# MarToonLi/StableDiffusionEO

Hardware: AMD Instinct MI355X
Metric: 512x512 canny2image images/sec (20 DDIM steps); ms per UNet step reported alongside (higher is better)
Workload: dtype f16; 1 GPU; SD1.5 + ControlNet-canny 512x512, batch=1 per GPU (CFG pair fused, N=2), 20 DDIM steps + VAE decode, fp16 storage / fp32 accumulate (BASELINE configs[1]); model_config=sd15, ddim_steps=20, parallelism=dp1 (image index -> rank, RCCL all_gather of final latents), weights=seeded synthetic (no checkpoint in the container)

## Files before the change

stablediffusioneo_amd/csrc/api_ops.hip:

```cpp
#include <stdarg.h>

#include "../../include/sdeo.h"
#include "sdeo_internal.h"
#include "kernels.h"

namespace sdeo {

static thread_local std::string g_last_error;

void set_error(const std::string& msg) { g_last_error = msg; }

int fail(const char* fmt, ...) {
  char buf[1024];
  va_list ap;
  va_start(ap, fmt);
  vsnprintf(buf, sizeof(buf), fmt, ap);
  va_end(ap);
  g_last_error = buf;
  return 1;
}

}

using namespace sdeo;
// ... 178 lines not shown
  (void)disarm_fp8();
  SDEO_CHECK(slots && groups > 0 && cout % groups == 0, "conv2d_gn: bad arguments");
  ConvGemm p;
  if (int rc = fill_conv(p, n, h, w, cin, cout, ksize, stride, upsample2x)) return rc;
  p.x = (const f16*)x; p.w = (const f16*)w_krsc; p.y = (f16*)y; p.bias = bias; p.res = (const f16*)res;
  p.bias2 = bias2; p.ld_bias2 = cout;
  const int cpg = cout / groups;
  *slots = conv_gemm_gn_slots(p, cpg);
  if (*slots <= 0) { *slots = 0; return 0; }
  const size_t need = (size_t)n * *slots * groups * 2, fold = *slots > 128 ? (size_t)n * groups * 2 : 0;
  SDEO_CHECK(partials && partial_floats >= need + fold, "conv2d_gn: partials buffer too small");
  p.gn_out = partials; p.gn_cpg = cpg; p.gn_slots = *slots; p.gn_groups = groups;
  if (int rc = conv_gemm(p, S(stream))) return rc;
  GnArgs g{(f16*)ynorm, (const f16*)y, gamma, beta, partials + need, cout, cout, n, p.Ho * p.Wo, cout, groups, eps, with_silu};
  g.ext_partials = partials; g.ext_nsc = *slots;
  return groupnorm_nhwc(g, S(stream));
}

static void fill_gemm(ConvGemm& p, int m, int n, int k) {
  p.B = m; p.Hi = p.Wi = p.Ho = p.Wo = 1; p.Cin = k; p.R = p.S = 1; p.stride = 1; p.pad = 0;
  p.M = m; p.N = n; p.K = k;
}

int sdeo_debug_gemm_plan(int m, int n, int k, int act, int fp8, int* key10, int* tile, int* splitk) {
  SDEO_CHECK(key10 && tile && splitk, "gemm_plan: null argument");
  ConvGemm p;
  fill_gemm(p, m, n, k);
  p.act = act;
  if (fp8) take_fp8(p, kQueryFp8);
  conv_gemm_query_plan(p, key10, tile, splitk);
// ... 280 lines not shown
```

stablediffusioneo_amd/csrc/kernels.h:

```cpp
#pragma once
#include <vector>

#include "common.h"

namespace sdeo {

struct ConvGemm {
  const f16* x = nullptr;
  const f16* w = nullptr;
  f16* y = nullptr;
  float* y32 = nullptr;
  const float* bias = nullptr;
  const float* bias2 = nullptr;
  const f16* res = nullptr;
  float* workspace = nullptr;
  size_t workspace_bytes = 0;
  int M = 0, N = 0, K = 0;
  int B = 1, Hi = 1, Wi = 1, Cin = 0;
  int Ho = 1, Wo = 1, R = 1, S = 1, stride = 1, pad = 0;
  int pad_after = -1;
  int ups = 0;
  int ldx = 0, ldw = 0, ldy = 0, ldres = 0, ld_bias2 = 0;
  int act = 0;
  int bias_per_row = 0;
// ... 55 lines not shown
int groupnorm_nhwc(f16* y, int ldy, const f16* x, int ldx, const float* gamma, const float* beta, int B, int HW, int C,
                   int groups, float eps, int with_silu, float* partials, hipStream_t stream);

struct GnArgs {
  f16* y; const f16* x; const float* gamma; const float* beta; float* partials;
  int ldy, ldx, B, HW, C, groups;
  float eps;
  int with_silu;
  const float* ext_partials = nullptr;
  int ext_nsc = 0;
};
bool groupnorm_is_single_launch(const GnArgs& a);
int gn_fused_threads(const GnArgs& a);
int groupnorm_nhwc(const GnArgs& a, hipStream_t stream);

int layernorm(f16* y, int ldy, const f16* x, int ldx, const float* gamma, const float* beta, int rows, int C, float eps,
              hipStream_t stream);

int attention(f16* o, int ldo, const f16* q, int ldq, const f16* k, int ldk, const f16* v, int ldv, int B, int H,
              int Tq, int Tk, int TkS, int TkSv, int d, float scale, hipStream_t stream, int causal = 0);
struct AttnArgs {
  f16* o; const f16* q; const f16* k; const f16* v;
  int ldo, ldq, ldk, ldv, B, H, Tq, Tk, TkS, TkSv, d;
  float scale;
  int causal;
  int qB = 0;
  int plan_B = 0;
};
int attention(const AttnArgs& a, hipStream_t stream);
const char* attention_kernel_name(int B, int H, int Tq, int Tk, int d, int causal);
// ... 74 lines not shown
```

stablediffusioneo_amd/csrc/net_build.hip:

```cpp
#include "net_handle.h"

namespace sdeo {

struct RowStats {
  float* p = nullptr;
  int ld = 0, strips = 0, c = 0;
};

struct ConvOpts {
  const float* bias2 = nullptr; int ld_bias2 = 0;
  const float* const* bias2_cur = nullptr; const int* ld_bias2_cur = nullptr; int bias2_off = 0;
  const T* res = nullptr;
  bool res_half = false;
  int act = 0;
  const float* scale_host = nullptr;
  const T* out = nullptr;
  int cout_store = -1;
  RowStats* stats = nullptr;
  const RowStats* ln = nullptr;
  const float* ln_s = nullptr;
  bool gn_next = false;
  const f16* w_ovr = nullptr; const float* b_ovr = nullptr;
  int pad_before = -1, pad_after = -1;
};

struct Builder {
  typedef ConvOpts CO;
  Engine* e;
  const Lane* lane;
  bool dry;
  bool share = false, half = false;
  Program* prog = nullptr;
  size_t max_splitk = 0, max_gn = 0;
  std::string err;

  T alloc(int n, int h, int w, int c) {
    T t;
    t.n = n; t.h = h; t.w = w; t.c = c; t.ld = c;
    t.off = lane->arena->alloc((size_t)n * h * w * c * 2);
    t.p = reinterpret_cast<f16*>(lane->base + t.off);
    return t;
  }
  T alloc2d(int rows, int c) { return alloc(1, 1, rows, c); }
  void release(T& t) { t.release(*lane->arena); }
  void advance(T& cur, T next) { release(cur); cur = next; }
  template <class F>
// ... 99 lines not shown
    T y = o.out ? o.out->view() : alloc(x.n, ho, wo, cs);
    const int n = half ? x.n / 2 : x.n;
    if (w && w->ipad != x.c && err.empty()) err = "conv " + name + ": input has " + std::to_string(x.c) + " channels, weight expects " + std::to_string(w->ipad);
    p.x = x.p; p.y = y.p;
    if (o.w_ovr) { p.w = o.w_ovr; p.bias = o.b_ovr; } else { p.w = wptr(name + ".weight"); p.bias = vptr(name + ".bias"); }
    p.bias2 = o.bias2; p.ld_bias2 = o.ld_bias2;
    if (o.res) { p.res = o.res->p; p.ldres = o.res->ld; }
    p.B = n; p.Hi = x.h; p.Wi = x.w; p.Cin = x.c; p.Ho = ho; p.Wo = wo; p.R = p.S = k; p.stride = stride; p.pad = pad; p.ups = ups;
    if (pad_after != pad) p.pad_after = pad_after;
    p.M = n * ho * wo; p.N = cs; p.K = k * k * x.c;
    if (half) p.plan_B = x.n;
    if (o.res_half) p.res_rows = p.M / 2;
    p.ldx = x.ld; p.ldw = p.K; p.ldy = y.ld; p.act = o.act;
    const bool want_gn = o.gn_next && !o.out && !o.scale_host && cs == y.c;
    if (want_gn) reserve_gn_partials(p, y);
    launch_conv(p, o.scale_host, o.stats, want_gn ? &y : nullptr, &o);
    return y;
  }

  T gemm(const T& x, const f16* w, int ldw, int n, const float* bias, const CO& o = CO(), float* out32 = nullptr, int ld32 = 0) {
    ConvGemm p;
    const int rows = half ? x.rows() / 2 : x.rows();
    T y;
    if (!out32) y = o.out ? o.out->view() : alloc(x.n, x.h, x.w, n);
    p.x = x.p; p.w = w; p.bias = bias;
    if (out32) { p.y32 = out32; p.ldy = ld32; } else { p.y = y.p; p.ldy = y.ld; }
    if (o.res) { p.res = o.res->p; p.ldres = o.res->ld; }
    p.B = rows; p.Cin = x.c; p.M = rows; p.N = n; p.K = x.c;
    p.ldx = x.ld; p.ldw = ldw; p.act = o.act;
    if (half) p.plan_B = x.rows();
    if (o.res_half) p.res_rows = rows / 2;
    set_ln(p, o);
// ... 21 lines not shown
    max_gn = std::max(max_gn, (size_t)B * gn_chunks(HW) * 32 * 2 * sizeof(float));
    const Lane* ws = lane;
    const f16* xp = x.p; f16* yp = y.p; const int ldx = x.ld, ldy = y.ld;
    GnArgs ga{yp, xp, g, b, nullptr, ldy, ldx, B, HW, C, 32, eps, silu_};
    const bool apply_only = x.gnp && !groupnorm_is_single_launch(ga);
    if (apply_only) {
      ga.ext_partials = x.gnp; ga.ext_nsc = x.gn_slots;
      max_gn = std::max(max_gn, (size_t)B * 32 * 2 * sizeof(float));
    }
    push([=](hipStream_t s) mutable { ga.partials = ws->gn_ws; return groupnorm_nhwc(ga, s); }, "groupnorm", 0,
         (apply_only ? 2.0 : 3.0) * 2.0 * B * HW * C, "C" + std::to_string(C) + " HW" + std::to_string(HW) + (apply_only ? " apply" : ""));
    return y;
  }

  T gn_conv(const T& x, const std::string& gn_name, float eps, int silu_, const std::string& conv_name, int cout, CO o) {
    T t = gn(x, gn_name, eps, silu_);
    T y = conv(t, conv_name, cout, 3, 1, 0, o);
    release(t);
    return y;
  }

  void attn(const T& o, const f16* q, int ldq, const f16* k, int ldk, const f16* v, int ldv, int B, int H, int Tq, int Tk, int TkS, int TkSv, int d,
            int qB = 0, const f16* k2 = nullptr, const f16* v2 = nullptr, int ldk2 = 0, int Tk2 = 0, int Tk2S = 0) {
    AttnArgs a{o.p, q, k, v, o.ld, ldq, ldk, ldv, B, H, Tq, Tk, TkS, TkSv, d, 1.0f / sqrtf((float)d), 0};
    a.qB = qB;
    if (half) { a.plan_B = B; a.B = B / 2; }
    B = a.B;
    const std::string tag = "Tq" + std::to_string(Tq) + " Tk" + std::to_string(Tk) + (k2 ? "+" + std::to_string(Tk2) : "") + " d" + std::to_string(d);
    if (k2) {
      if (!attention2_kernel_name(a.plan_B ? a.plan_B : a.B, H, Tq, Tk, Tk2, d) && err.empty()) err = std::string("image-prompt cross-attention: ") + sdeo_last_error();
      const Attn2Seg s2{k2, v2, ldk2, ldk2, Tk2, Tk2S, Tk2S, 0.f};
      const float* w = &e->ip_scale;
      push([=](hipStream_t s) { Attn2Seg x = s2; x.w = *w; return attention2(a, x, s); }, "attention",
           4.0 * B * H * (double)Tq * (Tk + Tk2) * d, 2.0 * B * H * d * (2.0 * Tq + 2.0 * (Tk + Tk2)), tag);
// ... 272 lines not shown
    if (i + 1 == e->hconvs.size()) o.out = &c.hint_feat[j];
    b.advance(x, b.conv(x, ns + hc.name, hc.cout, 3, hc.stride, 0, o));
  }
}

static T run_blocks(BuildCtx& c, const std::string& ns, const std::vector<Blk>& blocks, T x, bool release_in, int net, const T* final_out) {
  Builder& b = c.b;
  for (size_t i = 0; i < blocks.size(); ++i) {
    const Blk& blk = blocks[i];
    const T* out = (i + 1 == blocks.size()) ? final_out : nullptr;
    T y;
    switch (blk.kind) {
      case B_RES: y = build_res(b, ns, blk, x, net, out); break;
      case B_ATTN: y = build_attn(b, ns, blk, x, c.kv[net].at(ns + blk.name), net == 0 && b.e->ip_tokens ? &c.kv_ip.at(ns + blk.name) : nullptr, out); break;
      default: {
        Builder::CO o; o.out = out; o.gn_next = true;
        y = b.conv(x, ns + blk.name + conv_suffix(blk.kind), blk.cout, 3, blk.kind == B_DOWN ? 2 : 1, blk.kind == B_UP ? 1 : 0, o);
      }
    }
    if (release_in || i > 0) b.release(x);
    x = y;
  }
  return x;
}

struct Splice { size_t first = 0, last = 0; Program var; bool on = false; };
static T build_shared_prefix(BuildCtx& c, const std::string& ns, const std::vector<Blk>& blocks, const T& x, int net, Splice& sp) {
  Builder& b = c.b;
  Arena& arena = *b.lane->arena;
  const Arena before = arena;
  sp.first = b.prog->size();
// ... 24 lines not shown
  Builder& b = c.b; Engine* e = b.e;
  Splice sp;
  Program& p_cn = cn_prog(e, j, CP_CN);
  b.prog = &p_cn;
  const int net = 1 + j;
  const std::string ns = net_ns(net);
  auto zero_conv = [&](const T& x, const std::string& name, int cout, const T* out) {
    const size_t first = p_cn.size();
    Builder::CO zo; zo.out = out;
    b.conv(x, name, cout, 1, 1, 0, zo);
    for (size_t k = first; k < p_cn.size(); ++k) p_cn[k].zero_conv = true;
  };
  T hcur = e->x0;
  for (size_t i = 0; i < e->cplan.in.size(); ++i) {
    if (i == 0) {
      Builder::CO o; o.res = &c.hint_feat[j]; o.gn_next = true;
      hcur = b.conv(hcur, ns + e->cplan.in[0][0].name, e->cfg.model_channels, 3, 1, 0, o);
    } else if (i == 1) {
      hcur = build_shared_prefix(c, ns, e->cplan.in[i], hcur, net, sp);
    } else {
      hcur = run_blocks(c, ns, e->cplan.in[i], hcur, false, net, nullptr);
    }
    e->cn_h[j][i] = hcur;
    zero_conv(hcur, ns + "zero_convs." + std::to_string(i) + ".0", e->cplan.in_ch[i], &e->ctrl[i]);
  }
  T m = run_blocks(c, ns, e->cplan.mid, hcur, false, net, nullptr);
  e->cn_h[j][c.nctrl - 1] = m;
  zero_conv(m, ns + "middle_block_out.0", e->cplan.in_ch.back(), &e->ctrl[c.nctrl - 1]);
  splice(c, cn_prog(e, j, CP_CN_SH), p_cn, sp);
}

// ... 56 lines not shown
    }
    --ci;
    b.release(skip);
    const std::vector<Blk>& blocks = e->uplan.out[oi];
    if (oi + 1 < e->uplan.out.size()) {
      const T& nskip = hs.back();
      const int c_hn = blocks.back().cout;
      const int up = blocks.back().kind == B_UP ? 2 : 1;
      T ncat = b.alloc(cat.n, cat.h * up, cat.w * up, c_hn + nskip.c);
      const T nview = ncat.view(0, c_hn);
      run_blocks(c, ns, blocks, cat, true, 0, &nview);
      cat = ncat;
    } else {
      T y = run_blocks(c, ns, blocks, cat, true, 0, nullptr);
      Builder::CO oo; oo.cout_store = 4 * ((e->cfg.out_channels + 3) / 4);
      oo.out = &e->eps16;
      b.gn_conv(y, ns + "out.0", 1e-5f, 1, ns + "out.2", e->cfg.out_channels, oo);
      b.release(y);
    }
  }
}

static void build_unet_decoder_multi(BuildCtx& c, std::vector<T> hs, T cat0, T view0) {
  Builder& b = c.b; Engine* e = b.e;
  const std::string ns = NS_UNET;
  const size_t stages = e->uplan.out.size(), nh = hs.size();
  std::vector<T> cats{cat0};
  for (size_t oi = 0; oi + 1 < stages; ++oi) {
    const std::vector<Blk>& blocks = e->uplan.out[oi];
    const T& prev = cats.back();
    const int up = blocks.back().kind == B_UP ? 2 : 1;
// ... 21 lines not shown
  for (size_t oi = 0; oi < stages; ++oi, --ci) {
    const T& skip = hs[nh - 1 - oi];
    zero_conv(ci, "zero_convs." + std::to_string(ci) + ".0", cats[oi].view(cats[oi].c - skip.c, skip.c), skip);
  }
  if (!b.dry)
    for (int j = 0; j <= e->extra; ++j) b.prog->push_back(conv_gemm_multi_op(zc[j], kZeroConvTile, zs[j]));
  for (T& skip : hs) b.release(skip);
  for (size_t oi = 0; oi < stages; ++oi) {
    const std::vector<Blk>& blocks = e->uplan.out[oi];
    if (oi + 1 < stages) {
      const T nview = cats[oi + 1].view(0, blocks.back().cout);
      run_blocks(c, ns, blocks, cats[oi], true, 0, &nview);
    } else {
      T y = run_blocks(c, ns, blocks, cats[oi], true, 0, nullptr);
      Builder::CO oo; oo.cout_store = 4 * ((e->cfg.out_channels + 3) / 4);
      oo.out = &e->eps16;
      b.gn_conv(y, ns + "out.0", 1e-5f, 1, ns + "out.2", e->cfg.out_channels, oo);
      b.release(y);
    }
  }
}

static void build_unet(BuildCtx& c, bool with_ctrl) {
  Builder& b = c.b; Engine* e = b.e;
  b.prog = &e->prog[with_ctrl ? P_UNET_ENC : P_UNET_NOCTRL];
  const std::string ns = NS_UNET;
  std::vector<T> hs;
  T hcur = e->x0;
  Splice sp;
  for (size_t i = 0; i < e->uplan.in.size(); ++i) {
    hcur = (i == 1 && with_ctrl) ? build_shared_prefix(c, ns, e->uplan.in[i], hcur, 0, sp) : run_blocks(c, ns, e->uplan.in[i], hcur, false, 0, nullptr);
// ... 89 lines not shown
  b.advance(hcur, b.gn_conv(hcur, d + ".norm_out", 1e-6f, 1, d + ".conv_out", 2 * zc, oo));
  b.advance(hcur, b.conv(hcur, std::string(NS_VAE) + "quant_conv", 2 * zc, 1, 1, 0, oo));
  float* zp = e->enc_z; float* mp = e->enc_moments; const float* np_ = e->enc_noise; const int* with_noise = &e->enc_with_noise;
  const f16* qp = hcur.p; const int ld = hcur.ld, HW = h * w; const float sf = cfg.vae_scale_factor;
  b.push([=](hipStream_t s) { return vae_posterior(zp, mp, qp, ld, *with_noise ? np_ : nullptr, zc, HW, sf, s); }, "vae_posterior", 0,
         (2.0 * 2 * zc + 4.0 * 4 * zc) * HW);
  b.release(hcur);
}

}

int sdeo::build_all(Engine* e, bool dry, size_t* max_splitk, size_t* max_gn, size_t peaks[L_COUNT]) {
  Arena arenas[L_COUNT];
  for (int i = 0; i < L_COUNT; ++i) e->lanes[i].arena = &arenas[i];
  BuildCtx c{Builder{e, &e->lanes[L_MAIN], dry}, e->N, e->lh, e->lw, round8(e->cfg.context_len), (int)e->cplan.in.size() + 1};
  build_persistent(c);
  build_latent_io(c);
  build_time_embeds(c);
  for (int net = 0; net < 2 + e->extra; ++net) build_context(c, net);
  if (e->ip_tokens) build_context_ip(c);
  for (int j = 0; j <= e->extra; ++j) build_hint(c, j);
  c.b.on_lane(&e->lanes[L_SIDE], [&] { for (int j = 0; j <= e->extra; ++j) build_controlnet(c, j); });
  build_control_io(c);
  for (int variant = 0; variant < 2; ++variant) build_unet(c, variant == 0);
  build_vae_decoder(c);
  if (e->vae_encoder) build_vae_encoder(c);
  for (int i = 0; i < L_COUNT; ++i) {
    e->lanes[i].arena = nullptr;
    peaks[i] = align_up(arenas[i].peak, 256);
  }
// ... 5 lines not shown
```

stablediffusioneo_amd/csrc/norm.hip:

```cpp
#include <stdlib.h>

#include "kernels.h"

namespace sdeo {

struct GnOne {
  f16* y; const f16* x; const float* gamma; const float* beta; float* partials; int ldy, ldx;
};
struct GnPair { GnOne k[1]; };

int gn_chunks(int HW) { const int c = cdiv(HW, 8); return c > 128 ? 128 : (c < 1 ? 1 : c); }

static int gn_vec_per_block(int C, int groups) {
  const int nvec = C / 8, cpg = C / groups;
  for (int parts = 1; parts <= nvec; ++parts) {
    if (nvec % parts) continue;
    const int nvb = nvec / parts;
    if (nvb > 256) continue;
    if ((nvb * 8) % cpg) continue;
    return nvb;
  }
  return 0;
}

// ... 426 lines not shown
  if (chunks > 2048) chunks = 2048;
  const int ppc = cdiv(HW, chunks);
  dim3 grid(chunks, parts, B * count);
  int sc = cdiv(HW, 8 * P);
  { const int mxs = gn_chunks(HW) < 128 ? gn_chunks(HW) : 128; sc = sc < 1 ? 1 : (sc > mxs ? mxs : sc); }
  const int sppc = cdiv(HW, sc);
  dim3 sgrid(sc, parts, B * count);
  hipLaunchKernelGGL(gn_stats_kernel, sgrid, dim3(256), 0, stream, gp, B, HW, C, cpg, nvb, sc, groups, sppc);
  hipLaunchKernelGGL(gn_apply_kernel, grid, dim3(256), 0, stream, gp, B, HW, C, cpg, nvb, chunks, groups, eps, with_silu, ppc, sc);
  SDEO_HIP(hipGetLastError());
  return 0;
}

static GnOne gn_one(const GnArgs& a) { return GnOne{a.y, a.x, a.gamma, a.beta, a.partials, a.ldy, a.ldx}; }

int groupnorm_nhwc(const GnArgs& a, hipStream_t stream) {
  if (int rc = gn_check(a)) return rc;
  GnPair gp{};
  gp.k[0] = gn_one(a);
  return gn_dispatch(a, gp, 1, stream);
}

int groupnorm_nhwc(f16* y, int ldy, const f16* x, int ldx, const float* gamma, const float* beta, int B, int HW, int C,
                   int groups, float eps, int with_silu, float* partials, hipStream_t stream) {
  return groupnorm_nhwc(GnArgs{y, x, gamma, beta, partials, ldy, ldx, B, HW, C, groups, eps, with_silu}, stream);
}

template <int VPL>
__global__ __launch_bounds__(256) void layernorm_kernel(f16* __restrict__ y, int ldy, const f16* __restrict__ x, int ldx,
                                                        const float* __restrict__ gamma, const float* __restrict__ beta,
// ... 100 lines not shown
```

stablediffusioneo_amd/csrc/sdeo_internal.h:

```cpp
#ifndef SDEO_INTERNAL_H
#define SDEO_INTERNAL_H

#include <stdint.h>

#ifdef __cplusplus
extern "C" {
#endif

void sdeo_debug_force_gemm_plan(int tile, int splitk);
void sdeo_debug_force_gemm_order(int order);
const char* sdeo_debug_conv2d_kernel_name(int n, int h, int w, int cin, int cout, int ksize, int stride, int upsample2x);
const char* sdeo_debug_attention_kernel_name(int B, int H, int Tq, int Tk, int d, int causal);
const char* sdeo_debug_attention2_kernel_name(int B, int H, int Tq, int Tk, int Tk2, int d);
int sdeo_debug_attention2_check(void* o, int ldo, const void* q, int ldq, const void* k, int ldk, const void* v, int ldv, int tk, int tk_stride,
                                int v_batch_stride, const void* k2, int ldk2, const void* v2, int ldv2, int tk2, int tk2_stride,
                                int v2_batch_stride, float weight2, int b, int heads, int tq, int d, float scale);
int sdeo_debug_conv2d_plan(int n, int h, int w, int cin, int cout, int ksize, int stride, int upsample2x, int act, int fp8, int* key10,
                           int* tile, int* splitk);
int sdeo_debug_gemm_plan(int m, int n, int k, int act, int fp8, int* key10, int* tile, int* splitk);
int sdeo_debug_gemm_multi_f16(int count, const int* tile, const int* splitk, const int* m, const int* n, const int* k, void* const* y,
                              const int* ldy, const void* const* x, const int* ldx, const void* const* w, const int* ldw,
                              const void* const* bias, const void* const* res, const int* ldres, const float* scale, void* stream);
void sdeo_debug_last_gemm_plan(int* tile, int* splitk);
int sdeo_debug_last_gemm_epilogue(void);
// ... 17 lines not shown
int sdeo_debug_compose_proj(void* w_out, float* b_out, const void* wp, const float* bp, const void* w2, const float* b2, int c, int k2,
                            void* stream);
int sdeo_debug_gemm_stats_f16(void* y, int ldy, const void* x, int ldx, const void* w, int ldw, const float* bias, const void* res,
                              int ldres, int m, int n, int k, float* stats, int stats_ld, int* strips_out, void* stream);
int sdeo_debug_gemm_ln_f16(void* y, int ldy, const void* x, int ldx, const void* w_folded, int ldw, const float* ln_s,
                           const float* bias_folded, const float* stats, int stats_ld, int strips, int ln_c, int m, int n, int k, int act, float eps, void* workspace, size_t workspace_bytes, void* stream);
int sdeo_debug_row_stats_f16(float* stats, int stats_ld, const void* x, int ldx, int rows, int c, void* stream);
int sdeo_debug_conv2d_gn_f16(void* ynorm, void* y, const void* x, const void* w_krsc, const float* bias, const void* res, int n, int h,
                             int w, int cin, int cout, int ksize, int stride, int upsample2x, const float* gamma, const float* beta,
                             int groups, float eps, int with_silu, float* partials, size_t partial_floats, int* slots, void* stream);
int sdeo_debug_conv2d_gn_b2_f16(void* ynorm, void* y, const void* x, const void* w_krsc, const float* bias, const float* bias2, const void* res,
                                int n, int h, int w, int cin, int cout, int ksize, int stride, int upsample2x, const float* gamma,
                                const float* beta, int groups, float eps, int with_silu, float* partials, size_t partial_floats, int* slots,
                                void* stream);

int sdeo_debug_gemm_res_rows_f16(void* y, int ldy, const void* x, int ldx, const void* w, int ldw, const float* bias, const void* res,
                                 int ldres, int res_rows, int m, int n, int k, float* stats, int stats_ld, int* strips_out, void* workspace,
                                 size_t workspace_bytes, void* stream);
int sdeo_debug_conv2d_ex_f16(void* y, const void* x, const void* w_krsc, const float* bias, const void* res, int res_rows, int n, int h,
                             int w, int cin, int cout, int ksize, float* stats, int stats_ld, int* strips_out, const float* ln_stats,
                             const float* ln_s, int ln_ld, int ln_strips, void* workspace, size_t workspace_bytes, void* stream);
int sdeo_debug_attention_qb_f16(void* o, int ldo, const void* q, int ldq, const void* k, int ldk, const void* v, int ldv, int b,
                                int q_batches, int heads, int tq, int tk, int tk_stride, int v_batch_stride, int d, float scale, void* stream);
int sdeo_debug_attention2_qb_f16(void* o, int ldo, const void* q, int ldq, const void* k, int ldk, const void* v, int ldv, int tk,
                                 int tk_stride, int v_batch_stride, const void* k2, int ldk2, const void* v2, int ldv2, int tk2,
                                 int tk2_stride, int v2_batch_stride, float weight2, int b, int q_batches, int heads, int tq, int d,
                                 float scale, void* stream);

int sdeo_debug_quantize_mx(void* q_out, void* scales_out, const void* x, int rows, int cols, void* stream);
int sdeo_debug_gemm_mx_f16(void* y, int ldy, const void* xq, const void* xs, const void* wq, const void* ws, const float* bias, const void* res,
// ... 17 lines not shown
```

stablediffusioneo_amd/ops.py:

```python
from __future__ import annotations

import ctypes as C

import torch

from . import _lib
from ._lib import check, cur_stream, ptr


def _need_cuda(*ts):
    for t in ts:
        if t is not None and not t.is_cuda:
            raise _lib.SdeoError("HIP ops need device tensors (no CPU fallback)")


def _ws(nbytes, device):
    return torch.empty(max(int(nbytes), 16), dtype=torch.uint8, device=device)


def _nhwc_ld(t, what):
    n, h, w, _ = t.shape
    ld = t.stride(2)
    assert t.dtype == torch.float16 and t.stride(3) == 1 and (h == 1 or t.stride(1) == w * ld) and (n == 1 or t.stride(0) == h * w * ld), \
        f"groupnorm: {what} must be fp16 NHWC with unit channel stride and densely stacked pixels (shape {tuple(t.shape)}, strides {t.stride()})"
# ... 132 lines not shown
    hv, wv = (2 * h, 2 * w) if upsample2x else (h, w)
    pad = k // 2
    ho = (hv + 2 * pad - k) // stride + 1
    wo = (wv + 2 * pad - k) // stride + 1
    y = torch.empty((n, ho, wo, cout), dtype=torch.float16, device=x.device)
    yn = torch.empty_like(y)
    pf = n * (ho * wo) * groups * 2 // 16 + n * groups * 2 + 1024
    part = torch.empty(pf, dtype=torch.float32, device=x.device)
    slots = C.c_int(0)
    check(lib.sdeo_debug_conv2d_gn_f16(ptr(yn), ptr(y), ptr(x), ptr(w_krsc), ptr(bias), ptr(res), n, h, w, cin, cout, k, stride,
                                       int(upsample2x), ptr(gamma), ptr(beta), groups, eps, int(swish), ptr(part), pf, C.byref(slots),
                                       cur_stream()), "conv2d_gn")
    if slots.value == 0:
        return None
    return y, yn, slots.value


def gemm(x, w, bias=None, res=None, act=0, scale=1.0, out_f32=False, bias_per_row=False, w8=None, out=None):
    lib = _lib.load()
    _need_cuda(x, w)
    m, k = x.shape
    n, k2 = w.shape
    assert k == k2 and x.stride(1) == 1 and w.stride(1) == 1
    y = _out(out, (m, n), torch.float32 if out_f32 else torch.float16, x.device)
    nb = lib.sdeo_gemm_workspace_bytes(m, n, k)
    ws = _ws(nb if w8 is None else max(nb, 64 << 20), x.device)
    _arm_fp8(lib, w8)
    check(lib.sdeo_gemm_f16(ptr(y), n, ptr(x), x.stride(0), ptr(w), w.stride(0), ptr(bias), ptr(res),
                            res.stride(0) if res is not None else 0, m, n, k, act, scale, int(out_f32), int(bias_per_row), ptr(ws),
                            ws.numel(), cur_stream()), "gemm")
# ... 386 lines not shown
```

Baseline: 8.757 images/s.

## Add thin-channel conv kernels for UNet conv_in and fused GN-SiLU conv_out

Adds two specialised 3x3 conv kernels for the degenerate channel counts at the UNet and ControlNet edges. The first handles 4-to-8 stored input channels with the filter held in LDS and fdot2 accumulation, replacing the implicit-GEMM path. The second fuses GroupNorm finalisation, SiLU, and a 3x3 conv producing 4 output channels over a halo tile, with a cross-channel LDS reduction. Both are enabled by default through SDEO_THIN_CONVS. The goal is to avoid poorly utilised GEMM tiles and the separate normalised-tensor round trip, at the cost of new code paths and a large LDS footprint.

```diff
diff --git a/stablediffusioneo_amd/csrc/api_ops.hip b/stablediffusioneo_amd/csrc/api_ops.hip
--- a/stablediffusioneo_amd/csrc/api_ops.hip
+++ b/stablediffusioneo_amd/csrc/api_ops.hip
@@ -216,6 +216,31 @@
   if (int rc = conv_gemm(p, S(stream))) return rc;
   GnArgs g{(f16*)ynorm, (const f16*)y, gamma, beta, partials + need, cout, cout, n, p.Ho * p.Wo, cout, groups, eps, with_silu};
   g.ext_partials = partials; g.ext_nsc = *slots;
+  return groupnorm_nhwc(g, S(stream));
+}
+
+int sdeo_debug_conv3x3_cin4_f16(void* y, const void* x, const void* w_krsc, const float* bias, const void* res, int n_run, int h, int w, int cin,
+                                int cout, void* stream) {
+  const ThinConvIn a{(f16*)y, (const f16*)x, (const f16*)w_krsc, bias, (const f16*)res, cout, 8, 72, cout, n_run, h, w, cin, 8, cout};
+  return conv3x3_cin4(a, S(stream));
+}
+
+int sdeo_debug_gn_silu_conv3x3_cout4_f16(void* y, const void* x, const void* w_krsc, const float* bias, const float* gamma, const float* beta,
+                                         const float* partials, int slots, int n, int h, int w, int c, int cout, int groups, float eps,
+                                         int with_silu, void* workspace, void* stream) {
+  ThinConvOut a{(f16*)y, (const f16*)x, (const f16*)w_krsc, bias, gamma, beta, nullptr, 4, c, 9 * c, n, h, w, c, cout, groups, 0, eps, with_silu};
+  const char* why = gn_silu_conv3x3_cout4_refusal(a);
+  SDEO_CHECK(!why, "gn_silu_conv3x3_cout4: %s", why);
+  GnArgs g{nullptr, (const f16*)x, gamma, beta, (float*)workspace, c, c, n, h * w, c, groups, eps, with_silu};
+  if (partials) { g.ext_partials = partials; g.ext_nsc = slots; }
+  if (int rc = groupnorm_partials(g, &a.partials, &a.nsc, S(stream))) return rc;
+  return gn_silu_conv3x3_cout4(a, S(stream));
+}
+
+int sdeo_debug_groupnorm_from_partials_f16(void* y, const void* x, const float* gamma, const float* beta, const float* partials, int slots, int n,
+                                           int hw, int c, int groups, float eps, int with_silu, void* workspace, void* stream) {
+  GnArgs g{(f16*)y, (const f16*)x, gamma, beta, (float*)workspace, c, c, n, hw, c, groups, eps, with_silu};
+  g.ext_partials = partials; g.ext_nsc = slots;
   return groupnorm_nhwc(g, S(stream));
 }
 
diff --git a/stablediffusioneo_amd/csrc/conv_thin.hip b/stablediffusioneo_amd/csrc/conv_thin.hip
--- /dev/null
+++ b/stablediffusioneo_amd/csrc/conv_thin.hip
@@ -0,0 +1,341 @@
+#include "kernels.h"
+
+namespace sdeo {
+
+typedef _Float16 h2_t __attribute__((ext_vector_type(2)));
+typedef unsigned u32x4 __attribute__((ext_vector_type(4)));
+
+__device__ __forceinline__ float dot2(unsigned a, unsigned b, float c) {
+  return __builtin_amdgcn_fdot2(__builtin_bit_cast(h2_t, a), __builtin_bit_cast(h2_t, b), c, false);
+}
+
+template <int NP>
+struct PixVec { typedef unsigned type __attribute__((ext_vector_type(NP))); };
+
+template <int NP>
+__global__ __launch_bounds__(256) void conv3x3_cin4_kernel(const ThinConvIn a) {
+  kernarg_warm<sizeof(ThinConvIn)>();
+  typedef typename PixVec<NP>::type pix_t;
+  extern __shared__ __attribute__((aligned(16))) char thin_smem[];
+  pix_t* wl = reinterpret_cast<pix_t*>(thin_smem);
+  pix_t* tile = wl + a.Cout * 9;
+  const f16* __restrict__ x = a.x;
+  const f16* __restrict__ wgt = a.w;
+  const f16* __restrict__ res = a.res;
+  f16* __restrict__ y = a.y;
+  const int W = a.W, HW = a.H * a.W, L = a.L, ldx = a.ldx, ldy = a.ldy, ldres = a.ldres, ldw = a.ldw, cs = a.cin_store;
+  const int tid = threadIdx.x;
+  const int nvb = a.Cout >> 3, P = 256 / nvb;
+  const int cv = tid % nvb, prow = tid / nvb;
+  const bool active = prow < P;
+  const int b = blockIdx.y, p0 = blockIdx.x * L;
+  const int n = min(L, HW - p0);
+  const size_t img = (size_t)b * HW;
+
+#pragma unroll 4
+  for (int g = tid; g < a.Cout * 9; g += 256) {
+    const int row = g / 9, t = g - row * 9;
+    const u32x4 v = *reinterpret_cast<const u32x4*>(wgt + (size_t)row * ldw + t * cs);
+    pix_t o;
+#pragma unroll
+    for (int q = 0; q < NP; ++q) o[q] = v[q];
+    wl[((row & 7) * 9 + t) * nvb + (row >> 3)] = o;
+  }
+  const int nt = n + 2 * W + 2;
+  for (int i = tid; i < nt; i += 256) {
+    const int gp = p0 - W - 1 + i;
+    pix_t v = {};
+    if (gp >= 0 && gp < HW) v = *reinterpret_cast<const pix_t*>(x + (img + gp) * ldx);
+    tile[i] = v;
+  }
+  f32x4 bs[2] = {};
+  f16x8 rv[8];
+  if (active) {
+    if (a.bias) {
+      bs[0] = *reinterpret_cast<const f32x4*>(a.bias + cv * 8);
+      bs[1] = *reinterpret_cast<const f32x4*>(a.bias + cv * 8 + 4);
+    }
+    if (res) {
+#pragma unroll
+      for (int it = 0; it < 8; ++it) {
+        const int p = prow + it * P;
+        if (p < n) rv[it] = *reinterpret_cast<const f16x8*>(res + (img + p0 + p) * ldres + cv * 8);
+      }
+    }
+  }
+  __syncthreads();
+  if (!active) return;
+  pix_t w[8][9];
+#pragma unroll
+  for (int j = 0; j < 8; ++j)
+#pragma unroll
+    for (int t = 0; t < 9; ++t) w[j][t] = wl[(j * 9 + t) * nvb + cv];
+#pragma unroll
+  for (int it = 0; it < 8; ++it) {
+    const int p = prow + it * P;
+    if (p < n) {
+      const int xx = (p0 + p) % W;
+      float acc[8];
+#pragma unroll
+      for (int j = 0; j < 8; ++j) acc[j] = 0.f;
+#pragma unroll
+      for (int dy = 0; dy < 3; ++dy)
+#pragma unroll
+        for (int dx = 0; dx < 3; ++dx) {
+          pix_t v = tile[p + dy * W + dx];
+          if ((unsigned)(xx + dx - 1) >= (unsigned)W) v = pix_t{};
+#pragma unroll
+          for (int j = 0; j < 8; ++j)
+#pragma unroll
+            for (int q = 0; q < NP; ++q) acc[j] = dot2(v[q], w[j][dy * 3 + dx][q], acc[j]);
+        }
+      f16x8 o;
+#pragma unroll
+      for (int j = 0; j < 8; ++j) {
+        float f = acc[j] + bs[j >> 2][j & 3];
+        if (res) f += (float)rv[it][j];
+        o[j] = (f16)f;
+      }
+      *reinterpret_cast<f16x8*>(y + (img + p0 + p) * ldy + cv * 8) = o;
+    }
+  }
+}
+
+static int thin_conv_in_strip(const ThinConvIn& a) {
+  const int P = 256 / (a.Cout / 8), HW = a.H * a.W;
+  int L = cdiv(a.B * HW, 256);
+  L = L < P ? P : L;
+  L = L > 8 * P ? 8 * P : L;
+  L = L > 1024 ? 1024 : L;
+  return L > HW ? HW : L;
+}
+
+const char* conv3x3_cin4_refusal(const ThinConvIn& a) {
+  if (!a.y || !a.x || !a.w) return "null operand";
+  if (a.B < 1 || a.H < 1 || a.W < 1 || a.W > 1024) return "image size";
+  if (a.cin < 1 || a.cin > 8 || a.cin_store != 8 || a.ldw < 9 * a.cin_store) return "more than 8 stored input channels";
+  if (a.Cout < 8 || a.Cout % 8 || a.Cout > 384) return "output channels are no multiple of 8 (or above 384: the filter stays in LDS)";
+  if (a.ldx % 8 || a.ldy % 8 || a.ldw % 8 || (a.res && a.ldres % 8)) return "row strides are no multiples of 8";
+  if ((reinterpret_cast<uintptr_t>(a.x) | reinterpret_cast<uintptr_t>(a.y) | reinterpret_cast<uintptr_t>(a.w) | reinterpret_cast<uintptr_t>(a.res)) & 15)
+    return "operands are not 16-byte aligned";
+  if (a.bias && (reinterpret_cast<uintptr_t>(a.bias) & 15)) return "bias is not 16-byte aligned";
+  return nullptr;
+}
+
+int conv3x3_cin4(const ThinConvIn& a0, hipStream_t stream) {
+  const char* why = conv3x3_cin4_refusal(a0);
+  SDEO_CHECK(!why, "conv3x3_cin4: %s", why);
+  ThinConvIn a = a0;
+  a.L = thin_conv_in_strip(a);
+  const int HW = a.H * a.W, np = a.cin <= 4 ? 2 : 4;
+  const dim3 grid(cdiv(HW, a.L), a.B);
+  const size_t smem = (size_t)(a.Cout * 9 + a.L + 2 * a.W + 2) * np * 4;
+  SDEO_CHECK(smem <= 64 * 1024, "conv3x3_cin4: Cout=%d W=%d need %zu bytes of LDS", a.Cout, a.W, smem);
+  if (np == 2) hipLaunchKernelGGL(conv3x3_cin4_kernel<2>, grid, dim3(256), smem, stream, a);
+  else hipLaunchKernelGGL(conv3x3_cin4_kernel<4>, grid, dim3(256), smem, stream, a);
+  SDEO_HIP(hipGetLastError());
+  return 0;
+}
+
+static const int kThinPrefetch = 10;
+
+__global__ __launch_bounds__(256) void gn_silu_conv3x3_cout4_kernel(const ThinConvOut a) {
+  kernarg_warm<sizeof(ThinConvOut)>();
+  extern __shared__ __attribute__((aligned(16))) char thin_smem[];
+  const f16* __restrict__ x = a.x;
+  const f16* __restrict__ wgt = a.w;
+  const float* __restrict__ gamma = a.gamma;
+  const float* __restrict__ beta = a.beta;
+  const float* __restrict__ partials = a.partials;
+  f16* __restrict__ y = a.y;
+  const int H = a.H, W = a.W, C = a.C, ldx = a.ldx, ldw = a.ldw, TW = a.TW, TH = a.TH, groups = a.groups, nsc = a.nsc;
+  const int tid = threadIdx.x;
+  const int nvb = C >> 3, P = 256 / nvb;
+  const int cv = tid % nvb, prow = tid / nvb;
+  const bool active = prow < P;
+  const int b = blockIdx.y;
+  const int tx0 = (blockIdx.x % a.tiles_x) * TW, ty0 = (blockIdx.x / a.tiles_x) * TH;
+  const int HWD = TW + 2, HP = (TH + 2) * HWD, TP = TW * TH;
+  const int cpg = C / groups;
+  const int nab = C > 256 ? C : 256;
+  f16* halo = reinterpret_cast<f16*>(thin_smem);
+  f32x4* red = reinterpret_cast<f32x4*>(thin_smem + (size_t)HP * C * 2);
+  float* s_a = reinterpret_cast<float*>(red + (size_t)nvb * (TP + 1));
+  float* s_b = s_a + nab;
+  float* s_mean = s_b + nab;
+  float* s_rstd = s_mean + 64;
+  const f16* xb = x + (size_t)b * H * W * ldx + cv * 8;
+
+  f16x8 xv[kThinPrefetch];
+#pragma unroll
+  for (int u = 0; u < kThinPrefetch; ++u) {
+    const int hp = prow + u * P;
+    const int gy = ty0 + hp / HWD - 1, gx = tx0 + hp % HWD - 1;
+    xv[u] = f16x8{};
+    if (active && hp < HP && (unsigned)gy < (unsigned)H && (unsigned)gx < (unsigned)W)
+      xv[u] = *reinterpret_cast<const f16x8*>(xb + ((size_t)gy * W + gx) * ldx);
+  }
+  u32x4 w[4][9];
+#pragma unroll
+  for (int co = 0; co < 4; ++co)
+#pragma unroll
+    for (int t = 0; t < 9; ++t) {
+      w[co][t] = u32x4{};
+      if (active && co < a.cout) w[co][t] = *reinterpret_cast<const u32x4*>(wgt + (size_t)co * ldw + t * C + cv * 8);
+    }
+  float gpre[8], bpre[8];
+#pragma unroll
+  for (int k = 0; k < 8; ++k) {
+    const int c = tid + k * 256;
+    if (c < C) { gpre[k] = gamma[c]; bpre[k] = beta[c]; }
+  }
+  {
+    const int tpg = 256 / groups;
+    const int gl = tid / tpg, l = tid - gl * tpg;
+    float ts = 0.f, tq = 0.f;
+    if (gl < groups) {
+      const float2* src = reinterpret_cast<const float2*>(partials) + ((size_t)b * nsc * groups + gl);
+      for (int c0 = l; c0 < nsc; c0 += 8 * tpg) {
+        float2 v[8];
+#pragma unroll
+        for (int u = 0; u < 8; ++u) {
+          const int c = c0 + u * tpg;
+          v[u] = c < nsc ? src[(size_t)c * groups] : make_float2(0.f, 0.f);
+        }
+#pragma unroll
+        for (int u = 0; u < 8; ++u) { ts += v[u].x; tq += v[u].y; }
+      }
+    }
+    s_a[tid] = ts;
+    s_b[tid] = tq;
+  }
+  __syncthreads();
+  if (tid < groups) {
+    const int tpg = 256 / groups;
+    float ts = 0.f, tq = 0.f;
+    for (int l = 0; l < tpg; ++l) { ts += s_a[tid * tpg + l]; tq += s_b[tid * tpg + l]; }
+    const float inv = 1.0f / ((float)cpg * (float)(H * W));
+    const float mean = ts * inv;
+    float var = tq * inv - mean * mean;
+    var = var < 0.f ? 0.f : var;
+    s_mean[tid] = mean;
+    s_rstd[tid] = rsqrtf(var + a.eps);
+  }
+  __syncthreads();
+#pragma unroll
+  for (int k = 0; k < 8; ++k) {
+    const int c = tid + k * 256;
+    if (c < C) {
+      const int g = c / cpg;
+      const float sc = s_rstd[g] * gpre[k];
+      s_a[c] = sc;
+      s_b[c] = bpre[k] - s_mean[g] * sc;
+    }
+  }
+  __syncthreads();
+  if (active) {
+    float sa[8], sb[8];
+#pragma unroll
+    for (int j = 0; j < 8; ++j) { sa[j] = s_a[cv * 8 + j]; sb[j] = s_b[cv * 8 + j]; }
+    auto norm = [&](const f16x8& v, bool inside) {
+      f16x8 o;
+#pragma unroll
+      for (int j = 0; j < 8; ++j) {
+        float f = (float)v[j] * sa[j] + sb[j];
+        if (a.with_silu) f = silu_f(f);
+        o[j] = inside ? (f16)f : (f16)0.f;
+      }
+      return o;
+    };
+#pragma unroll
+    for (int u = 0; u < kThinPrefetch; ++u) {
+      const int hp = prow + u * P;
+      if (hp < HP) {
+        const int gy = ty0 + hp / HWD - 1, gx = tx0 + hp % HWD - 1;
+        *reinterpret_cast<f16x8*>(halo + (size_t)hp * C + cv * 8) = norm(xv[u], (unsigned)gy < (unsigned)H && (unsigned)gx < (unsigned)W);
+      }
+    }
+    for (int hp = prow + kThinPrefetch * P; hp < HP; hp += P) {
+      const int gy = ty0 + hp / HWD - 1, gx = tx0 + hp % HWD - 1;
+      const bool inside = (unsigned)gy < (unsigned)H && (unsigned)gx < (unsigned)W;
+      f16x8 v = {};
+      if (inside) v = *reinterpret_cast<const f16x8*>(xb + ((size_t)gy * W + gx) * ldx);
+      *reinterpret_cast<f16x8*>(halo + (size_t)hp * C + cv * 8) = norm(v, inside);
+    }
+  }
+  __syncthreads();
+  if (active) {
+    for (int p = prow; p < TP; p += P) {
+      const int py = p / TW, px = p - py * TW;
+      if (ty0 + py >= H || tx0 + px >= W) continue;
+      float acc[4] = {0.f, 0.f, 0.f, 0.f};
+#pragma unroll
+      for (int dy = 0; dy < 3; ++dy)
+#pragma unroll
+        for (int dx = 0; dx < 3; ++dx) {
+          const u32x4 v = *reinterpret_cast<const u32x4*>(halo + (size_t)((py + dy) * HWD + px + dx) * C + cv * 8);
+#pragma unroll
+          for (int co = 0; co < 4; ++co)
+#pragma unroll
+            for (int q = 0; q < 4; ++q) acc[co] = dot2(v[q], w[co][dy * 3 + dx][q], acc[co]);
+        }
+      red[(size_t)cv * (TP + 1) + p] = f32x4{acc[0], acc[1], acc[2], acc[3]};
+    }
+  }
+  __syncthreads();
+  if (tid < TP) {
+    const int py = tid / TW, px = tid - py * TW;
+    const int gy = ty0 + py, gx = tx0 + px;
+    if (gy < H && gx < W) {
+      f32x4 s = {0.f, 0.f, 0.f, 0.f};
+      for (int c = 0; c < nvb; ++c) s += red[(size_t)c * (TP + 1) + tid];
+      f16x4 o;
+#pragma unroll
+      for (int co = 0; co < 4; ++co) o[co] = co < a.cout ? (f16)(s[co] + (a.bias ? a.bias[co] : 0.f)) : (f16)0.f;
+      *reinterpret_cast<f16x4*>(y + (((size_t)b * H + gy) * W + gx) * a.ldy) = o;
+    }
+  }
+}
+
+static const size_t kThinOutLdsCap = 128 * 1024;
+
+static size_t thin_out_smem(int C, int TW, int TH) {
+  const int nvb = C / 8, HP = (TW + 2) * (TH + 2), TP = TW * TH, nab = C > 256 ? C : 256;
+  return (size_t)HP * C * 2 + (size_t)nvb * (TP + 1) * 16 + (size_t)(2 * nab + 128) * 4;
+}
+
+const char* gn_silu_conv3x3_cout4_refusal(const ThinConvOut& a) {
+  if (!a.y || !a.x || !a.w || !a.gamma || !a.beta) return "null operand";
+  if (a.B < 1 || a.H < 1 || a.W < 1) return "image size";
+  if (a.C < 8 || a.C % 8 || a.C > 512) return "channels are no multiple of 8 (or above 512)";
+  if (a.groups < 1 || a.groups > 64 || a.C % a.groups || 256 % a.groups) return "groups";
+  if (a.cout < 1 || a.cout > 4 || a.ldy % 4) return "more than 4 output channels";
+  if (a.ldx % 8 || a.ldw % 8 || a.ldw < 9 * a.C) return "row strides are no multiples of 8";
+  if ((reinterpret_cast<uintptr_t>(a.x) | reinterpret_cast<uintptr_t>(a.w)) & 15) return "operands are not 16-byte aligned";
+  if (reinterpret_cast<uintptr_t>(a.y) & 7) return "output is not 8-byte aligned";
+  return nullptr;
+}
+
+int gn_silu_conv3x3_cout4(const ThinConvOut& a0, hipStream_t stream) {
+  const char* why = gn_silu_conv3x3_cout4_refusal(a0);
+  SDEO_CHECK(!why, "gn_silu_conv3x3_cout4: %s", why);
+  SDEO_CHECK(a0.partials && a0.nsc >= 1 && a0.nsc <= 128, "gn_silu_conv3x3_cout4: bad statistics partials");
+  static DeviceOnce attr_done;
+  if (attr_done.need()) {
+    SDEO_HIP(hipFuncSetAttribute(reinterpret_cast<const void*>(&gn_silu_conv3x3_cout4_kernel), hipFuncAttributeMaxDynamicSharedMemorySize,
+                                 (int)kThinOutLdsCap));
+    attr_done.mark();
+  }
+  ThinConvOut a = a0;
+  a.TW = 8;
+  a.TH = a.B * cdiv(a.H, 8) * cdiv(a.W, 8) >= 256 ? 8 : 4;
+  a.tiles_x = cdiv(a.W, a.TW);
+  const int tiles_y = cdiv(a.H, a.TH);
+  const size_t smem = thin_out_smem(a.C, a.TW, a.TH);
+  SDEO_CHECK(smem <= kThinOutLdsCap, "gn_silu_conv3x3_cout4: C=%d needs %zu bytes of LDS", a.C, smem);
+  hipLaunchKernelGGL(gn_silu_conv3x3_cout4_kernel, dim3(a.tiles_x * tiles_y, a.B), dim3(256), smem, stream, a);
+  SDEO_HIP(hipGetLastError());
+  return 0;
+}
+
+}
diff --git a/stablediffusioneo_amd/csrc/kernels.h b/stablediffusioneo_amd/csrc/kernels.h
--- a/stablediffusioneo_amd/csrc/kernels.h
+++ b/stablediffusioneo_amd/csrc/kernels.h
@@ -93,6 +93,25 @@
 int gn_fused_threads(const GnArgs& a);
 int groupnorm_nhwc(const GnArgs& a, hipStream_t stream);
 
+int groupnorm_partials(const GnArgs& a, const float** partials, int* nsc, hipStream_t stream);
+
+struct ThinConvIn {
+  f16* y; const f16* x; const f16* w; const float* bias; const f16* res;
+  int ldy, ldx, ldw, ldres, B, H, W, cin, cin_store, Cout;
+  int L = 0;
+};
+const char* conv3x3_cin4_refusal(const ThinConvIn& a);
+int conv3x3_cin4(const ThinConvIn& a, hipStream_t stream);
+struct ThinConvOut {
+  f16* y; const f16* x; const f16* w; const float* bias; const float* gamma; const float* beta; const float* partials;
+  int ldy, ldx, ldw, B, H, W, C, cout, groups, nsc;
+  float eps;
+  int with_silu;
+  int TW = 0, TH = 0, tiles_x = 0;
+};
+const char* gn_silu_conv3x3_cout4_refusal(const ThinConvOut& a);
+int gn_silu_conv3x3_cout4(const ThinConvOut& a, hipStream_t stream);
+
 int layernorm(f16* y, int ldy, const f16* x, int ldx, const float* gamma, const float* beta, int rows, int C, float eps,
               hipStream_t stream);
 
diff --git a/stablediffusioneo_amd/csrc/net_build.hip b/stablediffusioneo_amd/csrc/net_build.hip
--- a/stablediffusioneo_amd/csrc/net_build.hip
+++ b/stablediffusioneo_amd/csrc/net_build.hip
@@ -22,6 +22,7 @@
   bool gn_next = false;
   const f16* w_ovr = nullptr; const float* b_ovr = nullptr;
   int pad_before = -1, pad_after = -1;
+  bool thin = false;
 };
 
 struct Builder {
@@ -30,6 +31,7 @@
   const Lane* lane;
   bool dry;
   bool share = false, half = false;
+  bool thin = true;
   Program* prog = nullptr;
   size_t max_splitk = 0, max_gn = 0;
   std::string err;
@@ -159,8 +161,22 @@
     p.ldx = x.ld; p.ldw = p.K; p.ldy = y.ld; p.act = o.act;
     const bool want_gn = o.gn_next && !o.out && !o.scale_host && cs == y.c;
     if (want_gn) reserve_gn_partials(p, y);
+    if (o.thin && thin_conv_in(p, o, w)) return y;
     launch_conv(p, o.scale_host, o.stats, want_gn ? &y : nullptr, &o);
     return y;
+  }
+
+  bool thin_allowed() const { return thin && e->fp8.weight_bits != 8 && e->fp8.act_bits != 8; }
+
+  bool thin_conv_in(const ConvGemm& p, const CO& o, const WEntry* w) {
+    if (!thin_allowed() || !w || p.R != 3 || p.stride != 1 || p.ups || p.pad != 1 || conv_pad_after(p) != 1 || o.act || o.bias2 || o.bias2_cur ||
+        o.scale_host || o.stats || o.ln || o.res_half)
+      return false;
+    const ThinConvIn a{p.y, p.x, p.w, p.bias, p.res, p.ldy, p.ldx, p.ldw, p.ldres, p.B, p.Hi, p.Wi, (int)w->dims[1], p.Cin, p.N};
+    if (conv3x3_cin4_refusal(a)) return false;
+    push([a](hipStream_t s) { return conv3x3_cin4(a, s); }, "conv_thin", 2.0 * p.M * p.N * 9 * a.cin, 2.0 * p.M * (p.N * (p.res ? 2 : 1) + p.Cin),
+         "in C" + std::to_string(p.N) + " HW" + std::to_string(p.Ho * p.Wo));
+    return true;
   }
 
   T gemm(const T& x, const f16* w, int ldw, int n, const float* bias, const CO& o = CO(), float* out32 = nullptr, int ld32 = 0) {
@@ -212,10 +228,48 @@
   }
 
   T gn_conv(const T& x, const std::string& gn_name, float eps, int silu_, const std::string& conv_name, int cout, CO o) {
+    if (o.thin) {
+      T y;
+      if (thin_conv_out(x, gn_name, eps, silu_, conv_name, cout, o, &y)) return y;
+    }
     T t = gn(x, gn_name, eps, silu_);
     T y = conv(t, conv_name, cout, 3, 1, 0, o);
     release(t);
     return y;
+  }
+
+  bool thin_conv_out(const T& x, const std::string& gn_name, float eps, int silu_, const std::string& conv_name, int cout, const CO& o, T* yo) {
+    const WEntry* w = W(conv_name + ".weight");
+    if (!thin_allowed() || !w || half || o.act || o.bias2 || o.bias2_cur || o.scale_host || o.stats || o.ln || o.res || o.w_ovr || o.gn_next ||
+        o.pad_before >= 0 || o.pad_after >= 0 || w->ipad != x.c || (int)w->dims[0] != cout || (int)w->dims[2] != 3)
+      return false;
+    const int cs = o.cout_store > 0 ? o.cout_store : cout;
+    if (cs != 4) return false;
+    const int B = x.n, HW = x.h * x.w, C = x.c;
+    ThinConvOut a{nullptr, x.p, wptr(conv_name + ".weight"), vptr(conv_name + ".bias"), vptr(gn_name + ".weight"), vptr(gn_name + ".bias"), nullptr,
+                  0, x.ld, 9 * C, B, x.h, x.w, C, cout, 32, 0, eps, silu_};
+    {
+      ThinConvOut q = a;
+      q.y = const_cast<f16*>(x.p); q.ldy = 4;
+      if (gn_silu_conv3x3_cout4_refusal(q)) return false;
+    }
+    T y = o.out ? o.out->view() : alloc(x.n, x.h, x.w, cs);
+    a.y = y.p; a.ldy = y.ld;
+    if (gn_silu_conv3x3_cout4_refusal(a)) {
+      if (err.empty()) err = std::string("conv ") + conv_name + ": " + gn_silu_conv3x3_cout4_refusal(a);
+      return false;
+    }
+    max_gn = std::max(max_gn, (size_t)B * gn_chunks(HW) * 32 * 2 * sizeof(float));
+    const Lane* ws = lane;
+    GnArgs ga{nullptr, x.p, a.gamma, a.beta, nullptr, x.ld, x.ld, B, HW, C, 32, eps, silu_};
+    if (x.gnp) { ga.ext_partials = x.gnp; ga.ext_nsc = x.gn_slots; }
+    push([=](hipStream_t s) mutable {
+      ga.partials = ws->gn_ws;
+      if (int rc = groupnorm_partials(ga, &a.partials, &a.nsc, s)) return rc;
+      return gn_silu_conv3x3_cout4(a, s);
+    }, "conv_thin", 2.0 * B * HW * 9 * C * cout, 2.0 * B * HW * (C + cs), "out C" + std::to_string(C) + " HW" + std::to_string(HW));
+    *yo = y;
+    return true;
   }
 
   void attn(const T& o, const f16* q, int ldq, const f16* k, int ldk, const f16* v, int ldv, int B, int H, int Tq, int Tk, int TkS, int TkSv, int d,
@@ -518,7 +572,7 @@
       case B_RES: y = build_res(b, ns, blk, x, net, out); break;
       case B_ATTN: y = build_attn(b, ns, blk, x, c.kv[net].at(ns + blk.name), net == 0 && b.e->ip_tokens ? &c.kv_ip.at(ns + blk.name) : nullptr, out); break;
       default: {
-        Builder::CO o; o.out = out; o.gn_next = true;
+        Builder::CO o; o.out = out; o.gn_next = true; o.thin = blk.kind == B_CONV_IN;
         y = b.conv(x, ns + blk.name + conv_suffix(blk.kind), blk.cout, 3, blk.kind == B_DOWN ? 2 : 1, blk.kind == B_UP ? 1 : 0, o);
       }
     }
@@ -573,7 +627,7 @@
   T hcur = e->x0;
   for (size_t i = 0; i < e->cplan.in.size(); ++i) {
     if (i == 0) {
-      Builder::CO o; o.res = &c.hint_feat[j]; o.gn_next = true;
+      Builder::CO o; o.res = &c.hint_feat[j]; o.gn_next = true; o.thin = true;
       hcur = b.conv(hcur, ns + e->cplan.in[0][0].name, e->cfg.model_channels, 3, 1, 0, o);
     } else if (i == 1) {
       hcur = build_shared_prefix(c, ns, e->cplan.in[i], hcur, net, sp);
@@ -660,7 +714,7 @@
     } else {
       T y = run_blocks(c, ns, blocks, cat, true, 0, nullptr);
       Builder::CO oo; oo.cout_store = 4 * ((e->cfg.out_channels + 3) / 4);
-      oo.out = &e->eps16;
+      oo.out = &e->eps16; oo.thin = true;
       b.gn_conv(y, ns + "out.0", 1e-5f, 1, ns + "out.2", e->cfg.out_channels, oo);
       b.release(y);
     }
@@ -712,7 +766,7 @@
     } else {
       T y = run_blocks(c, ns, blocks, cats[oi], true, 0, nullptr);
       Builder::CO oo; oo.cout_store = 4 * ((e->cfg.out_channels + 3) / 4);
-      oo.out = &e->eps16;
+      oo.out = &e->eps16; oo.thin = true;
       b.gn_conv(y, ns + "out.0", 1e-5f, 1, ns + "out.2", e->cfg.out_channels, oo);
       b.release(y);
     }
@@ -832,6 +886,7 @@
   Arena arenas[L_COUNT];
   for (int i = 0; i < L_COUNT; ++i) e->lanes[i].arena = &arenas[i];
   BuildCtx c{Builder{e, &e->lanes[L_MAIN], dry}, e->N, e->lh, e->lw, round8(e->cfg.context_len), (int)e->cplan.in.size() + 1};
+  { const char* v = getenv("SDEO_THIN_CONVS"); c.b.thin = !v || atoi(v) != 0; }
   build_persistent(c);
   build_latent_io(c);
   build_time_embeds(c);
diff --git a/stablediffusioneo_amd/csrc/norm.hip b/stablediffusioneo_amd/csrc/norm.hip
--- a/stablediffusioneo_amd/csrc/norm.hip
+++ b/stablediffusioneo_amd/csrc/norm.hip
@@ -464,6 +464,34 @@
 
 static GnOne gn_one(const GnArgs& a) { return GnOne{a.y, a.x, a.gamma, a.beta, a.partials, a.ldy, a.ldx}; }
 
+int groupnorm_partials(const GnArgs& a, const float** partials, int* nsc, hipStream_t stream) {
+  SDEO_CHECK(a.x && partials && nsc && (a.partials || (a.ext_partials && a.ext_nsc <= 128)), "groupnorm_partials: null operand");
+  SDEO_CHECK(a.B > 0 && a.HW > 0 && a.C > 0 && a.groups > 0 && a.groups <= 64 && a.C % a.groups == 0 && a.C % 8 == 0 && a.ldx % 8 == 0,
+             "groupnorm_partials: B=%d HW=%d C=%d groups=%d ldx=%d", a.B, a.HW, a.C, a.groups, a.ldx);
+  if (a.ext_partials) {
+    SDEO_CHECK(a.ext_nsc >= 1, "groupnorm_partials: bad producer partials");
+    *partials = a.ext_partials; *nsc = a.ext_nsc;
+    if (a.ext_nsc > 128) {
+      hipLaunchKernelGGL(gn_fold_partials_kernel, dim3(a.B * a.groups), dim3(256), 0, stream, reinterpret_cast<float2*>(a.partials),
+                         reinterpret_cast<const float2*>(a.ext_partials), a.ext_nsc, a.groups);
+      SDEO_HIP(hipGetLastError());
+      *partials = a.partials; *nsc = 1;
+    }
+    return 0;
+  }
+  const int nvb = gn_vec_per_block(a.C, a.groups);
+  SDEO_CHECK(nvb > 0, "groupnorm_partials: unsupported channel split C=%d groups=%d", a.C, a.groups);
+  const int parts = (a.C / 8) / nvb, P = 256 / nvb;
+  int sc = cdiv(a.HW, 8 * P);
+  { const int mxs = gn_chunks(a.HW) < 128 ? gn_chunks(a.HW) : 128; sc = sc < 1 ? 1 : (sc > mxs ? mxs : sc); }
+  GnPair gp{};
+  gp.k[0] = gn_one(a);
+  hipLaunchKernelGGL(gn_stats_kernel, dim3(sc, parts, a.B), dim3(256), 0, stream, gp, a.B, a.HW, a.C, a.C / a.groups, nvb, sc, a.groups, cdiv(a.HW, sc));
+  SDEO_HIP(hipGetLastError());
+  *partials = a.partials; *nsc = sc;
+  return 0;
+}
+
 int groupnorm_nhwc(const GnArgs& a, hipStream_t stream) {
   if (int rc = gn_check(a)) return rc;
   GnPair gp{};
diff --git a/stablediffusioneo_amd/csrc/sdeo_internal.h b/stablediffusioneo_amd/csrc/sdeo_internal.h
--- a/stablediffusioneo_amd/csrc/sdeo_internal.h
+++ b/stablediffusioneo_amd/csrc/sdeo_internal.h
@@ -55,6 +55,14 @@
                                 const float* beta, int groups, float eps, int with_silu, float* partials, size_t partial_floats, int* slots,
                                 void* stream);
 
+int sdeo_debug_conv3x3_cin4_f16(void* y, const void* x, const void* w_krsc, const float* bias, const void* res, int n_run, int h, int w, int cin,
+                                int cout, void* stream);
+int sdeo_debug_gn_silu_conv3x3_cout4_f16(void* y, const void* x, const void* w_krsc, const float* bias, const float* gamma, const float* beta,
+                                         const float* partials, int slots, int n, int h, int w, int c, int cout, int groups, float eps,
+                                         int with_silu, void* workspace, void* stream);
+int sdeo_debug_groupnorm_from_partials_f16(void* y, const void* x, const float* gamma, const float* beta, const float* partials, int slots, int n,
+                                           int hw, int c, int groups, float eps, int with_silu, void* workspace, void* stream);
+
 int sdeo_debug_gemm_res_rows_f16(void* y, int ldy, const void* x, int ldx, const void* w, int ldw, const float* bias, const void* res,
                                  int ldres, int res_rows, int m, int n, int k, float* stats, int stats_ld, int* strips_out, void* workspace,
                                  size_t workspace_bytes, void* stream);
diff --git a/stablediffusioneo_amd/ops.py b/stablediffusioneo_amd/ops.py
--- a/stablediffusioneo_amd/ops.py
+++ b/stablediffusioneo_amd/ops.py
@@ -170,6 +170,36 @@
     if slots.value == 0:
         return None
     return y, yn, slots.value
+
+
+def conv3x3_cin4(x, w_krsc, bias=None, res=None, cin=4, n_run=None, out=None):
+    lib = _lib.load()
+    _need_cuda(x, w_krsc)
+    n, h, w, cs = x.shape
+    cout = w_krsc.shape[0]
+    assert cs == 8 and tuple(w_krsc.shape[1:]) == (3, 3, 8) and x.is_contiguous() and w_krsc.is_contiguous()
+    assert res is None or (res.is_contiguous() and tuple(res.shape) == (n, h, w, cout))
+    y = _out(out, (n, h, w, cout), torch.float16, x.device)
+    check(lib.sdeo_debug_conv3x3_cin4_f16(ptr(y), ptr(x), ptr(w_krsc), ptr(bias), ptr(res), n if n_run is None else n_run, h, w, cin, cout,
+                                          cur_stream()), "conv3x3_cin4")
+    return y
+
+
+def gn_silu_conv3x3_cout4(x, w_krsc, gamma, beta, bias=None, groups=32, eps=1e-5, swish=True, partials=None):
+    lib = _lib.load()
+    _need_cuda(x, w_krsc, gamma, beta, partials)
+    n, h, w, c = x.shape
+    cout = w_krsc.shape[0]
+    assert tuple(w_krsc.shape[1:]) == (3, 3, c) and x.is_contiguous() and w_krsc.is_contiguous()
+    slots = 0
+    if partials is not None:
+        assert partials.dtype == torch.float32 and partials.is_contiguous() and partials.shape[0] == n and tuple(partials.shape[2:]) == (groups, 2)
+        slots = partials.shape[1]
+    ws = _ws(lib.sdeo_groupnorm_workspace_bytes(n, h * w, groups), x.device)
+    y = torch.empty((n, h, w, 4), dtype=torch.float16, device=x.device)
+    check(lib.sdeo_debug_gn_silu_conv3x3_cout4_f16(ptr(y), ptr(x), ptr(w_krsc), ptr(bias), ptr(gamma), ptr(beta), ptr(partials), slots, n, h, w,
+                                                   c, cout, groups, eps, int(swish), ptr(ws), cur_stream()), "gn_silu_conv3x3_cout4")
+    return y
 
 
 def gemm(x, w, bias=None, res=None, act=0, scale=1.0, out_f32=False, bias_per_row=False, w8=None, out=None):
```

Result: no change. 8.722 images/s (-0.4%).
